# KushalChaudhari-16/Medical-Image-Denoising-Using-Diffusion

Measured on AMD Instinct MI355X. Metric: denoised images/sec, 256x256 x50 DDIM steps, higher is better.
Workload: dtype f32 (split-fp16 x3 MFMA, fp32 accumulate); 1 GPU; batch=8/GPU 256x256 grayscale, 50-iteration reverse loop (noise_steps=50, inference_steps=50), random-init 12.8M-param UNet (BASELINE.json configs[1]); batch_per_gpu=8, global_batch=8, parallelism=single, collective=none

## Files before the change

include/midd.h:

```cpp
#ifndef MIDD_H
#define MIDD_H

#include <stddef.h>
#include <stdint.h>

#ifdef __cplusplus
extern "C" {
#endif

#define MI_OK            0
#define MI_EINVAL       -1
#define MI_ESTATE       -2
#define MI_EHIP         -3
#define MI_ENOMEM       -4
#define MI_ERANGE       -5

#define MI_STATUS_NONFINITE   1
#define MI_STATUS_FP16_RANGE  2

#define MI_MAX_LEVELS    8

#define MI_VARIANT_DDIM  0
#define MI_VARIANT_CDDPM 1

// ... 198 lines not shown

int mi_denoise_tiled_self_ensemble(mi_plan* plan, const float* noisy, float* mean_out, float* std_out, float* samples_out, float* tiles_out,
                                   int B, int H, int W, int th, int tw, int oy, int ox, const int32_t* views, int n_views,
                                   const int32_t* t_list, int n_iters,
                                   const float* beta, const float* alpha, const float* alpha_hat, int noise_steps,
                                   int seeded, uint64_t seed, int64_t sample_offset, int64_t member_offset, int pass_samples, int flags,
                                   const mi_update_rule* rule, void* workspace, size_t workspace_bytes, void* stream);

size_t mi_tiled_self_ensemble_workspace_bytes(mi_plan* plan, int B, int n_views, int H, int W, int th, int tw, int oy, int ox,
                                              int pass_samples, int tiles_external);

int mi_denoise_slots_rule(mi_plan* plan, const float* cond, float* x, int B, int H, int W,
                          const int32_t* t_rows, int n_rows, const int32_t* iter_base, const int64_t* sample_index,
                          const int64_t* member, const uint32_t* frame,
                          const int32_t* t_before, const int32_t* t_after, float* x0_hist,
                          const float* beta, const float* alpha, const float* alpha_hat, int noise_steps,
                          const float* step_noise, int seeded, uint64_t seed, int flags,
                          const mi_update_rule* rule, void* workspace, size_t workspace_bytes, void* stream);

int mi_status(const void* workspace, void* stream, int* flags);

int mi_debug_fetch(mi_plan* plan, const char* module_name, int B, int H, int W,
                   const void* workspace, float* dst, int* C, int* h, int* w, void* stream);

int mi_debug_attention_split(int N, int B, int* ksplit, int* tiles_per_split);

int mi_debug_plan_dump(mi_plan* plan, int B, int H, int W, int side_by_side, char* buf, size_t cap);

int mi_debug_conv16_geometry(int ks, int stride, int tw, int mt, int nt, int wm, int wn, int cb,
                             int* ring, int* ppw, int* apw, int* lds_bytes);
int mi_debug_conv16_geometry_planes(int ks, int stride, int tw, int mt, int nt, int wm, int wn, int cb, int planes,
                                    int* ring, int* ppw, int* apw, int* lds_bytes);
int mi_debug_conv16_steps(int Cin, int ks, int cb);

const char* mi_source_hash(void);

typedef struct mi_profile_entry {
    char   name[128];
    int64_t launches;
    double total_ms;
    double flops;
    double bytes;
} mi_profile_entry;
int mi_profile_begin(mi_plan* plan);
int mi_profile_end(mi_plan* plan, mi_profile_entry* out, int max_entries, int* n_entries);

int mi_noise_images(const float* clean, const int32_t* t, const float* alpha_hat, int noise_steps,
                    const float* eps, int seeded, uint64_t seed, int64_t sample_offset, int64_t draw,
                    const int64_t* sample_index, const int64_t* draws,
                    float* x_t, float* eps_out, int B, int C, int H, int W, void* stream);
size_t mi_loss_workspace_bytes(int B, int C, int H, int W);
int mi_loss_terms(const float* clean, const float* x_t, const float* eps, const float* eps_pred,
                  const int32_t* t, const float* alpha_hat, int noise_steps,
                  int seeded, uint64_t seed, int64_t sample_offset, int64_t draw,
                  const int64_t* sample_index, const int64_t* draws, int flags, double edge_weight,
                  double* out, float* maps, int B, int C, int H, int W,
                  void* workspace, size_t workspace_bytes, void* stream);
size_t mi_denoising_loss_workspace_bytes(mi_plan* plan, int B, int H, int W);
int mi_denoising_loss(mi_plan* plan, const float* clean, const float* cond, const int32_t* t,
                      const float* alpha_hat, int noise_steps,
                      const float* eps, int seeded, uint64_t seed, int64_t sample_offset, int64_t draw,
                      const int64_t* sample_index, const int64_t* draws, int flags, double edge_weight,
                      double* out, float* maps, int B, int H, int W,
                      void* workspace, size_t workspace_bytes, void* stream);

void mi_plan_destroy(mi_plan* plan);
// ... 37 lines not shown
```

medical-image-denoising-using-diffusion_amd/csrc/in_conv.hip:

```cpp
#include "midd_internal.h"
#include "pointwise_common.h"

namespace midd {

__global__ __launch_bounds__(256)
void in_conv_kernel(const float* __restrict__ x, const float* __restrict__ cond, const float* __restrict__ w,
                    const float* __restrict__ bias, float* __restrict__ out, stat_word* __restrict__ tot, int rep, int bs,
                    int ic, int H, int W, int Cout, int rows, int blocked) {
    extern __shared__ float wl[];
    const int nw = 9 * 2 * ic * Cout;
    for (int i = threadIdx.x; i < nw + Cout; i += 256) wl[i] = (i < nw) ? w[i] : bias[i - nw];
    __syncthreads();
    const int CG = Cout >> 4;
    const int ppi = 256 / CG;
    const int tid = threadIdx.x;
    const int pl = tid / CG, cg = tid - pl * CG;
    const bool active = pl < ppi;
    const int b = blockIdx.y, row = blockIdx.x;
    const int HW = H * W;
    const int per = (HW + rows - 1) / rows;
    const int p0 = row * per, p1 = min(HW, p0 + per);
    float ssum[16], ssq[16];
#pragma unroll
    for (int k = 0; k < 16; ++k) { ssum[k] = 0.f; ssq[k] = 0.f; }
// ... 19 lines not shown
#else
                        const float v = plane[(size_t)gy * W + gx];
#endif
                        const float* wr = &wl[((dy * 3 + dx) * 2 * ic + ci) * Cout + cg * 16];
#if defined(PW_ABL) && PW_ABL == 4
                        acc[dx] += v;
#else
#pragma unroll
                        for (int k = 0; k < 4; ++k) acc[k] += v * *reinterpret_cast<const f32x4*>(wr + k * 4);
#endif
                    }
                }
            }
#pragma unroll
            for (int k = 0; k < 4; ++k) {
#if defined(PW_ABL) && PW_ABL == 1
                if (acc[k][0] == 12345.678f)
#endif
                *reinterpret_cast<f32x4*>(out + act_index(blocked, b, Cout, HW, p, cg * 16 + k * 4)) = acc[k];
#if !(defined(PW_ABL) && PW_ABL == 2)
#pragma unroll
                for (int e = 0; e < 4; ++e) { ssum[k * 4 + e] += acc[k][e]; ssq[k * 4 + e] += acc[k][e] * acc[k][e]; }
#endif
            }
        }
    }
    if (tot == nullptr) return;
    float* const scratch = wl + nw + Cout;
    stat_word* const acc_lds = reinterpret_cast<stat_word*>(scratch + 2 * (size_t)Cout * ppi + (((nw + Cout) & 1) ? 1 : 0));
    pointwise_publish<16>(ssum, ssq, active, pl, ppi, cg, Cout, scratch, acc_lds, tot, b, bs, rep, row % rep, tid);
}

template <int COUT, bool BLOCKED>
__global__ __launch_bounds__(256, 3)
void in_conv1_kernel(const float* __restrict__ x, const float* __restrict__ cond, const float* __restrict__ w,
                     const float* __restrict__ bias, float* __restrict__ out, stat_word* __restrict__ tot, int rep, int bs,
                     int H, int W, int per) {
    constexpr int NQ = COUT / 4;
    constexpr int G64 = (NQ % 16 == 0) ? 16 : (NQ % 8 == 0) ? 8 : (NQ % 4 == 0) ? 4 : (NQ % 2 == 0) ? 2 : 1;
    constexpr int SETS = BLOCKED ? COUT / 16 : NQ / G64;
    constexpr int PS = COUT + 4;
    constexpr int SLOTS = BLOCKED ? 64 : 4 * SETS * ((64 + NQ - 1) / NQ);
    extern __shared__ __attribute__((aligned(16))) float ic1_lds[];
    const int tid = threadIdx.x, lane = tid & 63;
    const int wave = __builtin_amdgcn_readfirstlane(tid >> 6);
    float* const tile = ic1_lds + wave * (64 * PS);
    float* const wlds = ic1_lds + 4 * 64 * PS + ((COUT + 2) * STAT_WORDS * 2 + 4);
    for (int i = tid; i < 19 * COUT; i += 256) wlds[i] = (i < 18 * COUT) ? w[i] : bias[i - 18 * COUT];
    __syncthreads();
    const int b = blockIdx.y, HW = H * W;
    const int p0 = blockIdx.x * per, p1 = min(HW, p0 + per);
    const float* const xp = x + (size_t)b * HW;
    const float* const cp = cond + (size_t)b * HW;
    float ssum[SETS][4], ssq[SETS][4];
#pragma unroll
    for (int j = 0; j < SETS; ++j)
#pragma unroll
        for (int e = 0; e < 4; ++e) { ssum[j][e] = 0.f; ssq[j][e] = 0.f; }
    auto load_taps = [&](int base, float (&v)[18]) {
        const int pc = min(base + lane, HW - 1);
        const int oy = pc / W, ox = pc - oy * W;
#pragma unroll
        for (int dy = 0; dy < 3; ++dy) {
            const int gy = oy + dy - 1, cy = min(max(gy, 0), H - 1);
#pragma unroll
            for (int dx = 0; dx < 3; ++dx) {
                const int gx = ox + dx - 1, cx = min(max(gx, 0), W - 1);
                const bool in = (gy == cy) && (gx == cx);
#if defined(PW_ABL) && PW_ABL == 6
                const float a0 = (float)cx, a1 = (float)cy;
#else
                const float a0 = xp[cy * W + cx], a1 = cp[cy * W + cx];
#endif
                v[dy * 3 + dx] = in ? a0 : 0.f;
                v[9 + dy * 3 + dx] = in ? a1 : 0.f;
            }
        }
    };
    float vn[18];
    int base = p0 + wave * 64;
    if (base < p1) load_taps(base, vn);
    for (; base < p1; base += 256) {
        float v[18];
#pragma unroll
        for (int i = 0; i < 18; ++i) v[i] = vn[i];
        if (base + 256 < p1) load_taps(base + 256, vn);
        int wofs = 0;
        asm volatile("" : "+v"(wofs));
        const float* const wl = wlds + wofs;
        constexpr int NQH = NQ / 2;
#pragma unroll
        for (int h = 0; h < 2; ++h) {
            f32x4 acc[NQH], wv[2][NQH];
            auto wload = [&](int i, f32x4 (&d)[NQH]) {
#pragma unroll
                for (int q = 0; q < NQH; ++q) d[q] = *reinterpret_cast<const f32x4*>(wl + ((i % 9) * 2 + i / 9) * COUT + (h * NQH + q) * 4);
            };
#pragma unroll
            for (int q = 0; q < NQH; ++q) acc[q] = *reinterpret_cast<const f32x4*>(wl + 18 * COUT + (h * NQH + q) * 4);
            wload(0, wv[0]);
#pragma unroll
            for (int i = 0; i < 18; ++i) {
                if (i + 1 < 18) wload(i + 1, wv[(i + 1) & 1]);
                {
                    typedef float f32x2 __attribute__((ext_vector_type(2)));
                    f32x2 tp = {v[i], v[i]};
#pragma unroll
                    for (int q = 0; q < NQH; ++q) {
                        f32x2 a0 = {acc[q][0], acc[q][1]}, a1 = {acc[q][2], acc[q][3]};
                        const f32x2 w0 = {wv[i & 1][q][0], wv[i & 1][q][1]}, w1 = {wv[i & 1][q][2], wv[i & 1][q][3]};
                        asm volatile("v_pk_fma_f32 %0, %1, %2, %0 op_sel_hi:[1,0,1]" : "+v"(a0) : "v"(w0), "v"(tp));
                        asm volatile("v_pk_fma_f32 %0, %1, %2, %0 op_sel_hi:[1,0,1]" : "+v"(a1) : "v"(w1), "v"(tp));
                        acc[q] = (f32x4){a0[0], a0[1], a1[0], a1[1]};
                    }
                }
#pragma unroll
                for (int q = 0; q < NQH; ++q) asm volatile("" : "+v"(acc[q]));
            }
#pragma unroll
            for (int q = 0; q < NQH; ++q) *reinterpret_cast<f32x4*>(&tile[lane * PS + (h * NQH + q) * 4]) = acc[q];
        }
        const int npx = min(64, p1 - base);
#pragma unroll
        for (int r = 0; r < NQ; ++r) {
            int px, c, set; float* dst;
            if constexpr (BLOCKED) {
                const int k = r >> 2, idx = (r & 3) * 64 + lane;
                px = idx >> 2; c = k * 4 + (idx & 3); set = k;
                dst = out + (((size_t)b * (COUT / 16) + k) * HW + base) * 16 + (size_t)idx * 4;
            } else {
                const int idx = r * 64 + lane;
                px = idx / NQ; c = idx - px * NQ; set = r % SETS;
                dst = out + ((size_t)b * HW + base) * COUT + (size_t)idx * 4;
            }
            const f32x4 val = *reinterpret_cast<const f32x4*>(&tile[px * PS + c * 4]);
            if (px < npx) {
#if defined(PW_ABL) && PW_ABL == 5
                if (val[0] == 12345.678f)
#endif
                *reinterpret_cast<f32x4*>(dst) = val;
#pragma unroll
                for (int e = 0; e < 4; ++e) { ssum[set][e] += val[e]; ssq[set][e] += val[e] * val[e]; }
            }
        }
    }
    if (tot == nullptr) return;
#if defined(PW_ABL) && PW_ABL == 8
    if (ssum[0][0] != 12345.678f) return;
#endif
    __syncthreads();
    float* const scratch = ic1_lds;
    for (int i = tid; i < 2 * COUT * SLOTS; i += 256) scratch[i] = 0.f;
    __syncthreads();
#pragma unroll
    for (int j = 0; j < SETS; ++j) {
        const int quad = BLOCKED ? j * 4 + (lane & 3) : (lane + 64 * j) % NQ;
        const int slot = BLOCKED ? wave * 16 + (lane >> 2) : (wave * SETS + j) * ((64 + NQ - 1) / NQ) + lane / NQ;
#pragma unroll
        for (int e = 0; e < 4; ++e) {
            scratch[(size_t)(quad * 4 + e) * SLOTS + slot] = ssum[j][e];
            scratch[(size_t)(COUT + quad * 4 + e) * SLOTS + slot] = ssq[j][e];
        }
    }
    auto fold = [&](int i) {
        double t = 0;
        for (int l = 0; l < SLOTS; ++l) t += (double)scratch[(size_t)i * SLOTS + l];
        return (float)t;
    };
    stat_word* const acc_lds = reinterpret_cast<stat_word*>(ic1_lds + 4 * 64 * PS);
    stat_publish(tot, b, COUT, bs, rep, blockIdx.x % rep, 0, COUT, fold, acc_lds, tid, 256);
}

template <int COUT, bool BLOCKED>
static hipError_t in_conv1_launch(const float* x, const float* cond, const float* w, const float* bias, float* out,
                                  stat_word* tot, int rep, int bs, int B, int H, int W, hipStream_t s) {
#ifndef IC1_PASSES
#define IC1_PASSES 2
#endif
    const int HW = H * W;
    int per = IC1_PASSES * 256;
    while ((HW + per - 1) / per > 1024) per += 256;
    const int rows = (HW + per - 1) / per;
    constexpr int NQ = COUT / 4, PS = COUT + 4;
    constexpr int G64 = (NQ % 16 == 0) ? 16 : (NQ % 8 == 0) ? 8 : (NQ % 4 == 0) ? 4 : (NQ % 2 == 0) ? 2 : 1;
    constexpr int SLOTS = BLOCKED ? 64 : 4 * (NQ / G64) * ((64 + NQ - 1) / NQ);
    static_assert(2 * COUT * SLOTS <= 4 * 64 * PS, "the statistics scratch aliases the tiles");
    const size_t lds = (size_t)4 * 64 * PS * sizeof(float) + (size_t)(COUT + 2) * STAT_WORDS * sizeof(stat_word) + 16 + (size_t)19 * COUT * sizeof(float);
    {
        static int raised[MIDD_MAX_DEVICES] = {};
        hipError_t e = ensure_dynamic_lds(reinterpret_cast<const void*>(&in_conv1_kernel<COUT, BLOCKED>), (int)lds, raised);
        if (e != hipSuccess) return e;
    }
    hipLaunchKernelGGL((in_conv1_kernel<COUT, BLOCKED>), dim3(rows, B), dim3(256), lds, s, x, cond, w, bias, out, tot, rep, bs, H, W, per);
    return hipGetLastError();
}

hipError_t in_conv_launch(const float* x, const float* cond, const float* w, const float* bias, float* out,
                          stat_word* tot, int rep, int bs, int B, int ic, int H, int W, int Cout, int blocked, hipStream_t s) {
    if (Cout % 16 || Cout / 16 > 256) return hipErrorInvalidValue;
    if (ic == 1 && in_conv1_width(Cout)) {
#define MIDD_IC1(N) if (Cout == N) return blocked ? in_conv1_launch<N, true>(x, cond, w, bias, out, tot, rep, bs, B, H, W, s) \
                                                 : in_conv1_launch<N, false>(x, cond, w, bias, out, tot, rep, bs, B, H, W, s);
        MIDD_IC1(48) MIDD_IC1(32) MIDD_IC1(64)
        static_assert(in_conv1_width(48) && in_conv1_width(32) && in_conv1_width(64), "in_conv1_width names the instantiations");
#undef MIDD_IC1
    }
    const int ppi = 256 / (Cout / 16);
    const int rows = pointwise_rows(H * W, ppi);
    const size_t lds = in_conv_lds_bytes(ic, Cout);
    if (lds > POINTWISE_LDS_LIMIT) return hipErrorInvalidValue;
    hipLaunchKernelGGL(in_conv_kernel, dim3(rows, B), dim3(256), lds, s, x, cond, w, bias, out, tot, rep, bs, ic, H, W, Cout, rows, blocked);
    return hipGetLastError();
}

}
```

medical-image-denoising-using-diffusion_amd/csrc/midd_abi.hip:

```cpp
#include "midd_host.h"

using namespace midd;

static thread_local char g_err[512] = "";

int midd::fail(int code, const char* fmt, ...) {
    va_list ap;
    va_start(ap, fmt);
    vsnprintf(g_err, sizeof(g_err), fmt, ap);
    va_end(ap);
    return code;
}

extern "C" size_t mi_resize_workspace_bytes(int n, int sw, int sh, int dw, int dh) {
    if (n < 1 || sw < 1 || sh < 1 || dw < 1 || dh < 1) return 0;
    return resize_workspace_bytes(n, sw, sh, dw, dh);
}
extern "C" int mi_resize_bicubic_u8(const void* src, int n, int sw, int sh, void* dst, int dw, int dh,
                                    void* workspace, size_t workspace_bytes, void* stream) {
    if (!src || !dst || !workspace) return fail(MI_EINVAL, "null argument");
    if (n < 1 || sw < 1 || sh < 1 || dw < 1 || dh < 1) return fail(MI_EINVAL, "image sizes must be positive");
    if (reinterpret_cast<uintptr_t>(workspace) & 255) return fail(MI_EINVAL, "workspace must be 256-byte aligned");
    if (workspace_bytes < resize_workspace_bytes(n, sw, sh, dw, dh))
        return fail(MI_EINVAL, "workspace too small: %zu < %zu", workspace_bytes, resize_workspace_bytes(n, sw, sh, dw, dh));
// ... 201 lines not shown
    if (host & ~(MI_STATUS_NONFINITE | MI_STATUS_FP16_RANGE))
        return fail(MI_ERANGE, "status word 0x%x (bit 4: a -DMIDD_DMA_CHECK build saw an operand that had not landed when its counted wait returned)", host);
    if (host & MI_STATUS_FP16_RANGE)
        return fail(MI_ERANGE, "an attention operand exceeds the split-fp16 range (|q|, |k| or |v| >= 4094, or not finite): use compute=\"f32\"%s",
                    (host & MI_STATUS_NONFINITE) ? "; non-finite values reached later statistics" : "");
    if (host & MI_STATUS_NONFINITE) return fail(MI_ERANGE, "non-finite activations (NaN / Inf) reached a GroupNorm statistic or a raw operand");
    return MI_OK;
}

extern "C" int mi_debug_conv16_geometry(int ks, int stride, int tw, int mt, int nt, int wm, int wn, int cb, int* ring, int* ppw, int* apw, int* lds_bytes) {
    if (!ring || !ppw || !apw || !lds_bytes) return fail(MI_EINVAL, "null argument");
    ConvTile t{ks, stride, tw, mt, nt, wm, wn, cb};
    ConvLaunchInfo li{};
    if (!conv16_launch_info(384, 16 * nt * wn, 1, 64, 64, t, 0, &li)) return fail(MI_EINVAL, "tile (%d,%d,%d,%d,%d) ks %d stride %d cb %d is not instantiated", tw, mt, nt, wm, wn, ks, stride, cb);
    *ring = li.ring; *ppw = li.ppw; *apw = li.apw; *lds_bytes = li.lds_bytes;
    return MI_OK;
}
extern "C" int mi_debug_conv16_geometry_planes(int ks, int stride, int tw, int mt, int nt, int wm, int wn, int cb, int planes,
                                               int* ring, int* ppw, int* apw, int* lds_bytes) {
    if (!ring || !ppw || !apw || !lds_bytes) return fail(MI_EINVAL, "null argument");
    if (planes != 1 && planes != 2) return fail(MI_EINVAL, "planes must be 1 (f16) or 2 (f16x3), got %d", planes);
    ConvTile t{ks, stride, tw, mt, nt, wm, wn, cb, planes};
    ConvLaunchInfo li{};
    if (!conv16_launch_info(384, 16 * nt * wn, 1, 64, 64, t, 0, &li)) return fail(MI_EINVAL, "tile (%d,%d,%d,%d,%d) ks %d stride %d cb %d is not instantiated", tw, mt, nt, wm, wn, ks, stride, cb);
    *ring = li.ring; *ppw = li.ppw; *apw = li.apw; *lds_bytes = li.lds_bytes;
    return MI_OK;
}
extern "C" int mi_debug_conv16_steps(int Cin, int ks, int cb) {
    if (Cin < 16 || Cin % 16) return fail(MI_EINVAL, "Cin %d: a positive multiple of 16", Cin);
    if (ks != 1 && ks != 3) return fail(MI_EINVAL, "ks %d: 1 or 3", ks);
    if (cb < 0 || cb > 2 || (ks == 1 && cb == 1)) return fail(MI_EINVAL, "cb %d: 0 (default), 1 (3x3) or 2", cb);
    return conv16_num_steps(Cin, ks * ks, cb);
}
extern "C" int mi_debug_plan_dump(mi_plan* plan, int B, int H, int W, int side_by_side, char* buf, size_t cap) {
    if (!plan) return fail(MI_EINVAL, "null plan");
    std::string text;
    int rc = dump_program(plan, B, H, W, side_by_side != 0, &text);
    if (rc) return rc;
    if (buf && cap) { snprintf(buf, cap, "%s", text.c_str()); }
    return (int)text.size();
}

extern "C" void mi_plan_destroy(mi_plan* plan) {
    if (!plan) return;
    for (auto& sp : plan->spans) { (void)hipEventDestroy(sp.a); (void)hipEventDestroy(sp.b); }
    for (hipEvent_t ev : plan->event_pool) (void)hipEventDestroy(ev);
    if (plan->sev_fork) (void)hipEventDestroy(plan->sev_fork);
    for (int i = 0; i < mi_plan::MAX_PARTS; ++i) {
        if (plan->sev_phase[i]) (void)hipEventDestroy(plan->sev_phase[i]);
        if (plan->sev_join[i]) (void)hipEventDestroy(plan->sev_join[i]);
        if (plan->sstream[i]) (void)hipStreamDestroy(plan->sstream[i]);
    }
    if (plan->wdev) (void)hipFree(plan->wdev);
    if (plan->ttab) (void)hipFree(plan->ttab);
    delete plan;
}
```

medical-image-denoising-using-diffusion_amd/csrc/pointwise_common.h:

```cpp
#pragma once
#include "midd_internal.h"

namespace midd {

typedef float f32x4 __attribute__((ext_vector_type(4)));

static inline bool aligned16(const void* p) { return (reinterpret_cast<uintptr_t>(p) & 15) == 0; }

template <int NV>
__device__ __forceinline__ void pointwise_publish(const float (&sum)[NV], const float (&sq)[NV], bool active, int pl, int ppi, int cgrp,
                                                  int C, float* scratch, stat_word* acc, stat_word* tot, int b, int bs, int rep,
                                                  int replica, int tid, int nthreads = 256, int c0 = 0, int ncol = -1) {
    if (ncol < 0) ncol = C;
    if (active) {
#pragma unroll
        for (int e = 0; e < NV; ++e) {
            scratch[(size_t)(cgrp * NV + e) * ppi + pl] = sum[e];
            scratch[(size_t)(ncol + cgrp * NV + e) * ppi + pl] = sq[e];
        }
    }
    auto fold = [&](int i) {
        double t = 0;
        for (int l = 0; l < ppi; ++l) t += (double)scratch[(size_t)i * ppi + l];
        return (float)t;
    };
    stat_publish(tot, b, C, bs, rep, replica, c0, ncol, fold, acc, tid, nthreads);
}

static inline int pointwise_rows(int HW, int ppi) {
    int r = (HW + ppi * 4 - 1) / (ppi * 4);
    return r < 1 ? 1 : (r > 1024 ? 1024 : r);
}

__device__ __forceinline__ double add_rn64(double a, double b) {
#pragma clang fp contract(off)
    return a + b;
}
__device__ __forceinline__ double sub_rn64(double a, double b) {
#pragma clang fp contract(off)
    return a - b;
}
__device__ __forceinline__ double mul_rn64(double a, double b) {
#pragma clang fp contract(off)
    return a * b;
}

}
```

medical-image-denoising-using-diffusion_amd/csrc/resample.hip:

```cpp
#include "midd_internal.h"
#include "pointwise_common.h"

namespace midd {

__global__ __launch_bounds__(256)
void resize_bilinear_kernel(const float* __restrict__ src, float* __restrict__ dst, stat_word* __restrict__ tot, int rep, int bs,
                            int H, int W, int C, int OH, int OW, float sy, float sx, int rows) {
    extern __shared__ float rs_lds[];
    const int CQ = C >> 2;
    const int ppi = 256 / CQ;
    const int tid = threadIdx.x;
    const int pl = tid / CQ, cq = tid - pl * CQ;
    const bool active = pl < ppi;
    const int b = blockIdx.y, row = blockIdx.x;
    const int OHW = OH * OW;
    const int per = (OHW + rows - 1) / rows;
    const int p0 = row * per, p1 = min(OHW, p0 + per);
    float ssum[4] = {0.f, 0.f, 0.f, 0.f}, ssq[4] = {0.f, 0.f, 0.f, 0.f};
    if (active) {
        const float* base = src + (size_t)b * H * W * C + cq * 4;
        for (int p = p0 + pl; p < p1; p += ppi) {
            const int oy = p / OW, ox = p - oy * OW;
            float fy = sy * ((float)oy + 0.5f) - 0.5f; if (fy < 0.f) fy = 0.f;
            float fx = sx * ((float)ox + 0.5f) - 0.5f; if (fx < 0.f) fx = 0.f;
            const int y0 = (int)fy, x0 = (int)fx;
            const int y1 = y0 + (y0 < H - 1 ? 1 : 0), x1 = x0 + (x0 < W - 1 ? 1 : 0);
            const float ly1 = fy - (float)y0, lx1 = fx - (float)x0;
            const float ly0 = 1.0f - ly1, lx0 = 1.0f - lx1;
            const f32x4 v00 = *reinterpret_cast<const f32x4*>(base + ((size_t)y0 * W + x0) * C);
            const f32x4 v01 = *reinterpret_cast<const f32x4*>(base + ((size_t)y0 * W + x1) * C);
            const f32x4 v10 = *reinterpret_cast<const f32x4*>(base + ((size_t)y1 * W + x0) * C);
            const f32x4 v11 = *reinterpret_cast<const f32x4*>(base + ((size_t)y1 * W + x1) * C);
            const f32x4 r = ly0 * (lx0 * v00 + lx1 * v01) + ly1 * (lx0 * v10 + lx1 * v11);
            *reinterpret_cast<f32x4*>(dst + ((size_t)b * OHW + p) * C + cq * 4) = r;
#pragma unroll
            for (int e = 0; e < 4; ++e) { ssum[e] += r[e]; ssq[e] += r[e] * r[e]; }
        }
    }
    if (tot == nullptr) return;
    stat_word* const acc_lds = reinterpret_cast<stat_word*>(rs_lds + 2 * (size_t)C * ppi);
    pointwise_publish<4>(ssum, ssq, active, pl, ppi, cq, C, rs_lds, acc_lds, tot, b, bs, rep, row % rep, tid);
}

__global__ __launch_bounds__(256)
void resize_bilinear_blocked_kernel(const float* __restrict__ src, float* __restrict__ dst, stat_word* __restrict__ tot, int rep, int bs,
                                    int H, int W, int C, int OH, int OW, float sy, float sx, int rows) {
    __shared__ float rs_scratch[2 * 16 * 64];
    __shared__ stat_word rs_acc[(16 + 2) * STAT_WORDS];
    const int tid = threadIdx.x;
    const int pl = tid >> 2, q = tid & 3;
    const int b = blockIdx.y, row = blockIdx.x, blk = blockIdx.z;
    const int OHW = OH * OW;
    const int per = (OHW + rows - 1) / rows;
    const int p0 = row * per, p1 = min(OHW, p0 + per);
    float ssum[4] = {0.f, 0.f, 0.f, 0.f}, ssq[4] = {0.f, 0.f, 0.f, 0.f};
    const float* base = src + (((size_t)b * (C >> 4) + blk) * (size_t)(H * W)) * 16 + q * 4;
    float* const obase = dst + (((size_t)b * (C >> 4) + blk) * (size_t)OHW) * 16 + q * 4;
    for (int p = p0 + pl; p < p1; p += 64) {
        const int oy = p / OW, ox = p - oy * OW;
        float fy = sy * ((float)oy + 0.5f) - 0.5f; if (fy < 0.f) fy = 0.f;
        float fx = sx * ((float)ox + 0.5f) - 0.5f; if (fx < 0.f) fx = 0.f;
        const int y0 = (int)fy, x0 = (int)fx;
        const int y1 = y0 + (y0 < H - 1 ? 1 : 0), x1 = x0 + (x0 < W - 1 ? 1 : 0);
        const float ly1 = fy - (float)y0, lx1 = fx - (float)x0;
        const float ly0 = 1.0f - ly1, lx0 = 1.0f - lx1;
        const f32x4 v00 = *reinterpret_cast<const f32x4*>(base + ((size_t)y0 * W + x0) * 16);
        const f32x4 v01 = *reinterpret_cast<const f32x4*>(base + ((size_t)y0 * W + x1) * 16);
        const f32x4 v10 = *reinterpret_cast<const f32x4*>(base + ((size_t)y1 * W + x0) * 16);
        const f32x4 v11 = *reinterpret_cast<const f32x4*>(base + ((size_t)y1 * W + x1) * 16);
        const f32x4 r = ly0 * (lx0 * v00 + lx1 * v01) + ly1 * (lx0 * v10 + lx1 * v11);
        *reinterpret_cast<f32x4*>(obase + (size_t)p * 16) = r;
#pragma unroll
        for (int e = 0; e < 4; ++e) { ssum[e] += r[e]; ssq[e] += r[e] * r[e]; }
    }
    if (tot == nullptr) return;
    pointwise_publish<4>(ssum, ssq, true, pl, 64, q, C, rs_scratch, rs_acc, tot, b, bs, rep, row % rep, tid, 256, blk * 16, 16);
}

hipError_t resize_bilinear_launch(const float* src, float* dst, stat_word* tot, int rep, int bs, int B, int H, int W, int C, int OH, int OW, int blocked, hipStream_t s) {
    if (blocked) {
        if (C % 16) return hipErrorInvalidValue;
        const int rows_b = pointwise_rows(OH * OW, 64);
        hipLaunchKernelGGL(resize_bilinear_blocked_kernel, dim3(rows_b, B, C / 16), dim3(256), 0, s,
                           src, dst, tot, rep, bs, H, W, C, OH, OW, (float)H / (float)OH, (float)W / (float)OW, rows_b);
        return hipGetLastError();
    }
    if (C % 4 || C / 4 > 256) return hipErrorInvalidValue;
    const int ppi = 256 / (C / 4);
    const int rows = pointwise_rows(OH * OW, ppi);
    const size_t lds = (size_t)2 * C * ppi * sizeof(float) + (size_t)(C + 2) * STAT_WORDS * sizeof(stat_word);
    if (lds > 64 * 1024) return hipErrorInvalidValue;
    hipLaunchKernelGGL(resize_bilinear_kernel, dim3(rows, B), dim3(256), lds, s,
                       src, dst, tot, rep, bs, H, W, C, OH, OW, (float)H / (float)OH, (float)W / (float)OW, rows);
    return hipGetLastError();
}

__global__ __launch_bounds__(256)
void conv_transpose_kernel(const float* __restrict__ src, const float* __restrict__ w, const float* __restrict__ bias,
                           float* __restrict__ dst, int B, int H, int W, int Cin, int Cout, int blocked) {
    const int OH = 2 * H, OW = 2 * W, CQ = Cout >> 2;
    const long total = (long)B * OH * OW * CQ;
    const long gid = (long)blockIdx.x * 256 + threadIdx.x;
    if (gid >= total) return;
    const int cq = (int)(gid % CQ);
    const long pix = gid / CQ;
    const int ox = (int)(pix % OW);
    const int oy = (int)((pix / OW) % OH);
    const int b = (int)(pix / ((long)OW * OH));
    f32x4 acc = *reinterpret_cast<const f32x4*>(bias + cq * 4);
    for (int ky = 0; ky < 4; ++ky) {
        const int ny = oy + 1 - ky;
        if (ny < 0 || (ny & 1) || (ny >> 1) >= H) continue;
        for (int kx = 0; kx < 4; ++kx) {
            const int nx = ox + 1 - kx;
            if (nx < 0 || (nx & 1) || (nx >> 1) >= W) continue;
// ... 54 lines not shown
```

medical-image-denoising-using-diffusion_amd/native.py:

```python
from __future__ import annotations

import ctypes as C
import os
import threading

_HERE = os.path.dirname(os.path.abspath(__file__))
LIB_PATH = os.environ.get("MIDD_LIBRARY") or os.path.join(_HERE, "libmidd.so")

MI_MAX_LEVELS = 8
MI_VARIANT = {"ddim": 0, "cddpm": 1}
MI_CLAMP_EPS = 1
MI_NO_SPLIT = 2
MI_COMPUTE = {"f32": 0, "f16x3": 1, "f16": 2}
MI_STATUS_NONFINITE, MI_STATUS_FP16_RANGE = 1, 2
MI_COMPUTE_BATCH_INVARIANT = 0x100
MI_UPDATE = {"reference": 0, "ddim": 1, "dpmpp2m": 2}
MI_PIX_U8, MI_PIX_U16, MI_PIX_F32 = 0, 1, 2


class NativeLibraryError(RuntimeError):
    pass


class MiddError(RuntimeError):
# ... 93 lines not shown
    ("mi_denoise_rule", C.c_int, [C.c_void_p, C.c_void_p, C.c_void_p, C.c_int, C.c_int, C.c_int,
                                  C.POINTER(C.c_int32), C.c_int, C.POINTER(C.c_float), C.POINTER(C.c_float),
                                  C.POINTER(C.c_float), C.c_int, C.c_void_p, C.c_int, C.c_uint64, C.c_int64, C.c_int,
                                  C.POINTER(UpdateRule), C.c_void_p, C.c_size_t, C.c_void_p]),
    ("mi_denoise_ensemble_rule", C.c_int, [C.c_void_p, C.c_void_p, C.c_void_p, C.c_void_p, C.c_void_p, C.c_int, C.c_int, C.c_int, C.c_int,
                                           C.POINTER(C.c_int32), C.c_int, C.POINTER(C.c_float), C.POINTER(C.c_float),
                                           C.POINTER(C.c_float), C.c_int, C.c_uint64, C.c_int64, C.c_int64, C.c_int, C.c_int,
                                           C.POINTER(UpdateRule), C.c_void_p, C.c_size_t, C.c_void_p]),
    ("mi_denoise_tiled_rule", C.c_int, [C.c_void_p, C.c_void_p, C.c_void_p, C.c_void_p] + [C.c_int] * 7 +
                                       [C.POINTER(C.c_int32), C.c_int, C.POINTER(C.c_float), C.POINTER(C.c_float), C.POINTER(C.c_float), C.c_int,
                                        C.c_int, C.c_uint64, C.c_int64, C.c_int, C.c_int, C.POINTER(UpdateRule), C.c_void_p, C.c_size_t, C.c_void_p]),
    ("mi_dpm_coefficients", C.c_int, [C.POINTER(C.c_int32), C.c_int, C.POINTER(C.c_float), C.c_int, C.POINTER(C.c_float)]),
    ("mi_denoise_dpm", C.c_int, [C.c_void_p, C.c_void_p, C.c_void_p, C.c_void_p, C.c_int, C.c_int, C.c_int, C.c_int,
                                 C.POINTER(C.c_int32), C.c_int, C.POINTER(C.c_float), C.POINTER(C.c_float),
                                 C.POINTER(C.c_float), C.c_int, C.c_int, C.c_int, C.c_void_p, C.c_size_t, C.c_void_p]),
    ("mi_denoise_tiled_dpm", C.c_int, [C.c_void_p, C.c_void_p, C.c_void_p, C.c_void_p, C.c_void_p] + [C.c_int] * 7 +
                                      [C.POINTER(C.c_int32), C.c_int, C.POINTER(C.c_float), C.POINTER(C.c_float), C.POINTER(C.c_float), C.c_int,
                                       C.c_int, C.c_int, C.c_int, C.c_void_p, C.c_size_t, C.c_void_p]),
    ("mi_update_row", C.c_int, [C.c_int32, C.c_int32, C.c_int32, C.POINTER(C.c_float), C.c_int, C.c_double, C.POINTER(C.c_float)]),
    ("mi_denoise_slots_rule", C.c_int, [C.c_void_p, C.c_void_p, C.c_void_p, C.c_int, C.c_int, C.c_int,
                                        C.POINTER(C.c_int32), C.c_int, C.POINTER(C.c_int32), C.POINTER(C.c_int64),
                                        C.POINTER(C.c_int64), C.POINTER(C.c_uint32),
                                        C.POINTER(C.c_int32), C.POINTER(C.c_int32), C.c_void_p,
                                        C.POINTER(C.c_float), C.POINTER(C.c_float), C.POINTER(C.c_float), C.c_int,
                                        C.c_void_p, C.c_int, C.c_uint64, C.c_int, C.POINTER(UpdateRule), C.c_void_p, C.c_size_t, C.c_void_p]),
    ("mi_debug_fetch", C.c_int, [C.c_void_p, C.c_char_p, C.c_int, C.c_int, C.c_int, C.c_void_p, C.c_void_p,
                                 C.POINTER(C.c_int), C.POINTER(C.c_int), C.POINTER(C.c_int), C.c_void_p]),
    ("mi_status", C.c_int, [C.c_void_p, C.c_void_p, C.POINTER(C.c_int)]),
    ("mi_debug_attention_split", C.c_int, [C.c_int, C.c_int, C.POINTER(C.c_int), C.POINTER(C.c_int)]),
    ("mi_debug_plan_dump", C.c_int, [C.c_void_p, C.c_int, C.c_int, C.c_int, C.c_int, C.c_char_p, C.c_size_t]),
    ("mi_debug_conv16_geometry", C.c_int, [C.c_int] * 8 + [C.POINTER(C.c_int)] * 4),
    ("mi_debug_conv16_geometry_planes", C.c_int, [C.c_int] * 9 + [C.POINTER(C.c_int)] * 4),
    ("mi_debug_conv16_steps", C.c_int, [C.c_int] * 3),
    ("mi_source_hash", C.c_char_p, []),
    ("mi_profile_begin", C.c_int, [C.c_void_p]),
    ("mi_profile_end", C.c_int, [C.c_void_p, C.POINTER(ProfileEntry), C.c_int, C.POINTER(C.c_int)]),
    ("mi_resize_workspace_bytes", C.c_size_t, [C.c_int, C.c_int, C.c_int, C.c_int, C.c_int]),
    ("mi_resize_bicubic_u8", C.c_int, [C.c_void_p, C.c_int, C.c_int, C.c_int, C.c_void_p, C.c_int, C.c_int,
                                       C.c_void_p, C.c_size_t, C.c_void_p]),
    ("mi_u8_to_unit_f32", C.c_int, [C.c_void_p, C.c_void_p, C.c_size_t, C.c_void_p]),
    ("mi_unit_f32_to_u8", C.c_int, [C.c_void_p, C.c_void_p, C.c_size_t, C.c_void_p]),
    ("mi_resize_f32_workspace_bytes", C.c_size_t, [C.c_int, C.c_int, C.c_int, C.c_int, C.c_int]),
    ("mi_resize_bicubic_f32", C.c_int, [C.c_void_p, C.c_int, C.c_int, C.c_int, C.c_int, C.c_void_p, C.c_int, C.c_int, C.c_int, C.c_int,
                                        C.c_void_p, C.c_size_t, C.c_void_p]),
    ("mi_u16_to_unit_f32", C.c_int, [C.c_void_p, C.c_void_p, C.c_size_t, C.c_void_p]),
    ("mi_unit_f32_to_u16", C.c_int, [C.c_void_p, C.c_void_p, C.c_size_t, C.c_void_p]),
    ("mi_histogram_u16", C.c_int, [C.c_void_p, C.c_int, C.c_size_t, C.c_void_p, C.c_void_p]),
    ("mi_window_levels", C.c_int, [C.c_void_p, C.c_int, C.c_double, C.c_double, C.c_void_p, C.c_void_p]),
    ("mi_window_u16_to_f32", C.c_int, [C.c_void_p, C.c_void_p, C.c_int, C.c_size_t, C.c_void_p, C.c_void_p]),
    ("mi_window_f32_to_u16", C.c_int, [C.c_void_p, C.c_void_p, C.c_int, C.c_size_t, C.c_void_p, C.c_void_p]),
    ("mi_resize_bicubic_f32_window", C.c_int, [C.c_void_p, C.c_int, C.c_int, C.c_int, C.c_int, C.c_void_p, C.c_int, C.c_int, C.c_int,
                                               C.c_int, C.c_void_p, C.c_void_p, C.c_size_t, C.c_void_p]),
    ("mi_metrics_workspace_bytes", C.c_size_t, [C.c_int, C.c_int]),
    ("mi_image_metrics", C.c_int, [C.c_void_p, C.c_void_p, C.c_int, C.c_int, C.c_int, C.c_void_p,
                                   C.c_void_p, C.c_size_t, C.c_void_p]),
    ("mi_noise_images", C.c_int, [C.c_void_p, C.POINTER(C.c_int32), C.POINTER(C.c_float), C.c_int, C.c_void_p, C.c_int, C.c_uint64, C.c_int64,
                                  C.c_int64, C.POINTER(C.c_int64), C.POINTER(C.c_int64), C.c_void_p, C.c_void_p] + [C.c_int] * 4 + [C.c_void_p]),
    ("mi_loss_workspace_bytes", C.c_size_t, [C.c_int] * 4),
    ("mi_loss_terms", C.c_int, [C.c_void_p] * 4 + [C.POINTER(C.c_int32), C.POINTER(C.c_float), C.c_int, C.c_int, C.c_uint64, C.c_int64, C.c_int64,
                                C.POINTER(C.c_int64), C.POINTER(C.c_int64), C.c_int, C.c_double, C.c_void_p, C.c_void_p] + [C.c_int] * 4 + [C.c_void_p, C.c_size_t, C.c_void_p]),
    ("mi_denoising_loss_workspace_bytes", C.c_size_t, [C.c_void_p, C.c_int, C.c_int, C.c_int]),
    ("mi_denoising_loss", C.c_int, [C.c_void_p] * 3 + [C.POINTER(C.c_int32), C.POINTER(C.c_float), C.c_int, C.c_void_p, C.c_int, C.c_uint64, C.c_int64,
                                    C.c_int64, C.POINTER(C.c_int64), C.POINTER(C.c_int64), C.c_int, C.c_double, C.c_void_p, C.c_void_p] + [C.c_int] * 3 + [C.c_void_p, C.c_size_t, C.c_void_p]),
    ("mi_plan_destroy", None, [C.c_void_p]),
    ("mi_last_error", C.c_char_p, []),
    ("mi_version", C.c_char_p, []),
# ... 47 lines not shown
```

Measured before the change: 51.09 images/s.

## Add banded 2x bilinear upsample path and dual-strip blocked first conv

Adds a specialized path for exact 2x bilinear upsampling in the blocked layout. Each block processes a band of output rows and reuses horizontally interpolated source rows held in registers, instead of recomputing the taps for every output pixel. The blocked first-conv kernel now processes two 64-pixel strips per wave so each LDS weight load is shared across both strips; its occupancy bound drops from 3 to 2 to make room for the extra registers. The statistics scratch stride is padded to an odd value to avoid LDS bank conflicts, and a debug entry point for the resize kernel is exposed.

```diff
diff --git a/include/midd.h b/include/midd.h
--- a/include/midd.h
+++ b/include/midd.h
@@ -254,6 +254,9 @@
 int mi_debug_conv16_geometry_planes(int ks, int stride, int tw, int mt, int nt, int wm, int wn, int cb, int planes,
                                     int* ring, int* ppw, int* apw, int* lds_bytes);
 int mi_debug_conv16_steps(int Cin, int ks, int cb);
+
+int mi_debug_resize_bilinear(const float* src, float* dst, uint64_t* totals, int rep, int bs, int B, int H, int W, int C,
+                             int OH, int OW, void* stream);
 
 const char* mi_source_hash(void);
 
diff --git a/medical-image-denoising-using-diffusion_amd/csrc/in_conv.hip b/medical-image-denoising-using-diffusion_amd/csrc/in_conv.hip
--- a/medical-image-denoising-using-diffusion_amd/csrc/in_conv.hip
+++ b/medical-image-denoising-using-diffusion_amd/csrc/in_conv.hip
@@ -75,7 +75,7 @@
 }
 
 template <int COUT, bool BLOCKED>
-__global__ __launch_bounds__(256, 3)
+__global__ __launch_bounds__(256, BLOCKED ? 2 : 3)
 void in_conv1_kernel(const float* __restrict__ x, const float* __restrict__ cond, const float* __restrict__ w,
                      const float* __restrict__ bias, float* __restrict__ out, stat_word* __restrict__ tot, int rep, int bs,
                      int H, int W, int per) {
@@ -120,70 +120,139 @@
             }
         }
     };
-    float vn[18];
-    int base = p0 + wave * 64;
-    if (base < p1) load_taps(base, vn);
-    for (; base < p1; base += 256) {
-        float v[18];
-#pragma unroll
-        for (int i = 0; i < 18; ++i) v[i] = vn[i];
-        if (base + 256 < p1) load_taps(base + 256, vn);
-        int wofs = 0;
-        asm volatile("" : "+v"(wofs));
-        const float* const wl = wlds + wofs;
-        constexpr int NQH = NQ / 2;
-#pragma unroll
-        for (int h = 0; h < 2; ++h) {
-            f32x4 acc[NQH], wv[2][NQH];
-            auto wload = [&](int i, f32x4 (&d)[NQH]) {
-#pragma unroll
-                for (int q = 0; q < NQH; ++q) d[q] = *reinterpret_cast<const f32x4*>(wl + ((i % 9) * 2 + i / 9) * COUT + (h * NQH + q) * 4);
-            };
-#pragma unroll
-            for (int q = 0; q < NQH; ++q) acc[q] = *reinterpret_cast<const f32x4*>(wl + 18 * COUT + (h * NQH + q) * 4);
-            wload(0, wv[0]);
-#pragma unroll
-            for (int i = 0; i < 18; ++i) {
-                if (i + 1 < 18) wload(i + 1, wv[(i + 1) & 1]);
-                {
-                    typedef float f32x2 __attribute__((ext_vector_type(2)));
-                    f32x2 tp = {v[i], v[i]};
-#pragma unroll
-                    for (int q = 0; q < NQH; ++q) {
-                        f32x2 a0 = {acc[q][0], acc[q][1]}, a1 = {acc[q][2], acc[q][3]};
-                        const f32x2 w0 = {wv[i & 1][q][0], wv[i & 1][q][1]}, w1 = {wv[i & 1][q][2], wv[i & 1][q][3]};
-                        asm volatile("v_pk_fma_f32 %0, %1, %2, %0 op_sel_hi:[1,0,1]" : "+v"(a0) : "v"(w0), "v"(tp));
-                        asm volatile("v_pk_fma_f32 %0, %1, %2, %0 op_sel_hi:[1,0,1]" : "+v"(a1) : "v"(w1), "v"(tp));
-                        acc[q] = (f32x4){a0[0], a0[1], a1[0], a1[1]};
+    if constexpr (BLOCKED) {
+        constexpr int NB = COUT / 16;
+        float vn[2][18];
+        int base = p0 + wave * 64;
+        if (base < p1) { load_taps(base, vn[0]); load_taps(base + 256, vn[1]); }
+        for (; base < p1; base += 512) {
+            float v[2][18];
+#pragma unroll
+            for (int s = 0; s < 2; ++s)
+#pragma unroll
+                for (int i = 0; i < 18; ++i) v[s][i] = vn[s][i];
+            if (base + 512 < p1) { load_taps(base + 512, vn[0]); load_taps(base + 768, vn[1]); }
+            int wofs = 0;
+            asm volatile("" : "+v"(wofs));
+            const float* const wl = wlds + wofs;
+#pragma unroll
+            for (int k = 0; k < NB; ++k) {
+                f32x4 acc[2][4], wv[2][4];
+                auto wload = [&](int i, f32x4 (&d)[4]) {
+#pragma unroll
+                    for (int q = 0; q < 4; ++q) d[q] = *reinterpret_cast<const f32x4*>(wl + ((i % 9) * 2 + i / 9) * COUT + (k * 4 + q) * 4);
+                };
+#pragma unroll
+                for (int q = 0; q < 4; ++q) acc[0][q] = acc[1][q] = *reinterpret_cast<const f32x4*>(wl + 18 * COUT + (k * 4 + q) * 4);
+                wload(0, wv[0]);
+#pragma unroll
+                for (int i = 0; i < 18; ++i) {
+                    if (i + 1 < 18) wload(i + 1, wv[(i + 1) & 1]);
+#pragma unroll
+                    for (int s = 0; s < 2; ++s) {
+                        typedef float f32x2 __attribute__((ext_vector_type(2)));
+                        f32x2 tp = {v[s][i], v[s][i]};
+#pragma unroll
+                        for (int q = 0; q < 4; ++q) {
+                            f32x2 a0 = {acc[s][q][0], acc[s][q][1]}, a1 = {acc[s][q][2], acc[s][q][3]};
+                            const f32x2 w0 = {wv[i & 1][q][0], wv[i & 1][q][1]}, w1 = {wv[i & 1][q][2], wv[i & 1][q][3]};
+                            asm volatile("v_pk_fma_f32 %0, %1, %2, %0 op_sel_hi:[1,0,1]" : "+v"(a0) : "v"(w0), "v"(tp));
+                            asm volatile("v_pk_fma_f32 %0, %1, %2, %0 op_sel_hi:[1,0,1]" : "+v"(a1) : "v"(w1), "v"(tp));
+                            acc[s][q] = (f32x4){a0[0], a0[1], a1[0], a1[1]};
+                        }
                     }
-                }
-#pragma unroll
-                for (int q = 0; q < NQH; ++q) asm volatile("" : "+v"(acc[q]));
-            }
-#pragma unroll
-            for (int q = 0; q < NQH; ++q) *reinterpret_cast<f32x4*>(&tile[lane * PS + (h * NQH + q) * 4]) = acc[q];
-        }
-        const int npx = min(64, p1 - base);
-#pragma unroll
-        for (int r = 0; r < NQ; ++r) {
-            int px, c, set; float* dst;
-            if constexpr (BLOCKED) {
-                const int k = r >> 2, idx = (r & 3) * 64 + lane;
-                px = idx >> 2; c = k * 4 + (idx & 3); set = k;
-                dst = out + (((size_t)b * (COUT / 16) + k) * HW + base) * 16 + (size_t)idx * 4;
-            } else {
-                const int idx = r * 64 + lane;
-                px = idx / NQ; c = idx - px * NQ; set = r % SETS;
-                dst = out + ((size_t)b * HW + base) * COUT + (size_t)idx * 4;
-            }
-            const f32x4 val = *reinterpret_cast<const f32x4*>(&tile[px * PS + c * 4]);
-            if (px < npx) {
+#pragma unroll
+                    for (int s = 0; s < 2; ++s)
+#pragma unroll
+                        for (int q = 0; q < 4; ++q) asm volatile("" : "+v"(acc[s][q]));
+                }
+#pragma unroll
+                for (int s = 0; s < 2; ++s) {
+                    const int sbase = base + 256 * s, npx = min(64, p1 - sbase);
+#pragma unroll
+                    for (int q = 0; q < 4; ++q) *reinterpret_cast<f32x4*>(&tile[lane * PS + (k * 4 + q) * 4]) = acc[s][q];
+#pragma unroll
+                    for (int r4 = 0; r4 < 4; ++r4) {
+                        const int idx = r4 * 64 + lane, px = idx >> 2, c = k * 4 + (idx & 3);
+                        const f32x4 val = *reinterpret_cast<const f32x4*>(&tile[px * PS + c * 4]);
+                        if (px < npx) {
 #if defined(PW_ABL) && PW_ABL == 5
-                if (val[0] == 12345.678f)
-#endif
-                *reinterpret_cast<f32x4*>(dst) = val;
-#pragma unroll
-                for (int e = 0; e < 4; ++e) { ssum[set][e] += val[e]; ssq[set][e] += val[e] * val[e]; }
+                            if (val[0] == 12345.678f)
+#endif
+                            *reinterpret_cast<f32x4*>(out + (((size_t)b * NB + k) * HW + sbase) * 16 + (size_t)idx * 4) = val;
+#pragma unroll
+                            for (int e = 0; e < 4; ++e) { ssum[k][e] += val[e]; ssq[k][e] += val[e] * val[e]; }
+                        }
+                    }
+                }
+            }
+        }
+    } else {
+        float vn[18];
+        int base = p0 + wave * 64;
+        if (base < p1) load_taps(base, vn);
+        for (; base < p1; base += 256) {
+            float v[18];
+#pragma unroll
+            for (int i = 0; i < 18; ++i) v[i] = vn[i];
+            if (base + 256 < p1) load_taps(base + 256, vn);
+            int wofs = 0;
+            asm volatile("" : "+v"(wofs));
+            const float* const wl = wlds + wofs;
+            constexpr int NQH = NQ / 2;
+#pragma unroll
+            for (int h = 0; h < 2; ++h) {
+                f32x4 acc[NQH], wv[2][NQH];
+                auto wload = [&](int i, f32x4 (&d)[NQH]) {
+#pragma unroll
+                    for (int q = 0; q < NQH; ++q) d[q] = *reinterpret_cast<const f32x4*>(wl + ((i % 9) * 2 + i / 9) * COUT + (h * NQH + q) * 4);
+                };
+#pragma unroll
+                for (int q = 0; q < NQH; ++q) acc[q] = *reinterpret_cast<const f32x4*>(wl + 18 * COUT + (h * NQH + q) * 4);
+                wload(0, wv[0]);
+#pragma unroll
+                for (int i = 0; i < 18; ++i) {
+                    if (i + 1 < 18) wload(i + 1, wv[(i + 1) & 1]);
+                    {
+                        typedef float f32x2 __attribute__((ext_vector_type(2)));
+                        f32x2 tp = {v[i], v[i]};
+#pragma unroll
+                        for (int q = 0; q < NQH; ++q) {
+                            f32x2 a0 = {acc[q][0], acc[q][1]}, a1 = {acc[q][2], acc[q][3]};
+                            const f32x2 w0 = {wv[i & 1][q][0], wv[i & 1][q][1]}, w1 = {wv[i & 1][q][2], wv[i & 1][q][3]};
+                            asm volatile("v_pk_fma_f32 %0, %1, %2, %0 op_sel_hi:[1,0,1]" : "+v"(a0) : "v"(w0), "v"(tp));
+                            asm volatile("v_pk_fma_f32 %0, %1, %2, %0 op_sel_hi:[1,0,1]" : "+v"(a1) : "v"(w1), "v"(tp));
+                            acc[q] = (f32x4){a0[0], a0[1], a1[0], a1[1]};
+                        }
+                    }
+#pragma unroll
+                    for (int q = 0; q < NQH; ++q) asm volatile("" : "+v"(acc[q]));
+                }
+#pragma unroll
+                for (int q = 0; q < NQH; ++q) *reinterpret_cast<f32x4*>(&tile[lane * PS + (h * NQH + q) * 4]) = acc[q];
+            }
+            const int npx = min(64, p1 - base);
+#pragma unroll
+            for (int r = 0; r < NQ; ++r) {
+                int px, c, set; float* dst;
+                if constexpr (BLOCKED) {
+                    const int k = r >> 2, idx = (r & 3) * 64 + lane;
+                    px = idx >> 2; c = k * 4 + (idx & 3); set = k;
+                    dst = out + (((size_t)b * (COUT / 16) + k) * HW + base) * 16 + (size_t)idx * 4;
+                } else {
+                    const int idx = r * 64 + lane;
+                    px = idx / NQ; c = idx - px * NQ; set = r % SETS;
+                    dst = out + ((size_t)b * HW + base) * COUT + (size_t)idx * 4;
+                }
+                const f32x4 val = *reinterpret_cast<const f32x4*>(&tile[px * PS + c * 4]);
+                if (px < npx) {
+#if defined(PW_ABL) && PW_ABL == 5
+                    if (val[0] == 12345.678f)
+#endif
+                    *reinterpret_cast<f32x4*>(dst) = val;
+#pragma unroll
+                    for (int e = 0; e < 4; ++e) { ssum[set][e] += val[e]; ssq[set][e] += val[e] * val[e]; }
+                }
             }
         }
     }
@@ -193,7 +262,8 @@
 #endif
     __syncthreads();
     float* const scratch = ic1_lds;
-    for (int i = tid; i < 2 * COUT * SLOTS; i += 256) scratch[i] = 0.f;
+    constexpr int SSTR = SLOTS | 1;
+    for (int i = tid; i < 2 * COUT * SSTR; i += 256) scratch[i] = 0.f;
     __syncthreads();
 #pragma unroll
     for (int j = 0; j < SETS; ++j) {
@@ -201,13 +271,13 @@
         const int slot = BLOCKED ? wave * 16 + (lane >> 2) : (wave * SETS + j) * ((64 + NQ - 1) / NQ) + lane / NQ;
 #pragma unroll
         for (int e = 0; e < 4; ++e) {
-            scratch[(size_t)(quad * 4 + e) * SLOTS + slot] = ssum[j][e];
-            scratch[(size_t)(COUT + quad * 4 + e) * SLOTS + slot] = ssq[j][e];
+            scratch[(size_t)(quad * 4 + e) * SSTR + slot] = ssum[j][e];
+            scratch[(size_t)(COUT + quad * 4 + e) * SSTR + slot] = ssq[j][e];
         }
     }
     auto fold = [&](int i) {
         double t = 0;
-        for (int l = 0; l < SLOTS; ++l) t += (double)scratch[(size_t)i * SLOTS + l];
+        for (int l = 0; l < SLOTS; ++l) t += (double)scratch[(size_t)i * SSTR + l];
         return (float)t;
     };
     stat_word* const acc_lds = reinterpret_cast<stat_word*>(ic1_lds + 4 * 64 * PS);
@@ -227,7 +297,7 @@
     constexpr int NQ = COUT / 4, PS = COUT + 4;
     constexpr int G64 = (NQ % 16 == 0) ? 16 : (NQ % 8 == 0) ? 8 : (NQ % 4 == 0) ? 4 : (NQ % 2 == 0) ? 2 : 1;
     constexpr int SLOTS = BLOCKED ? 64 : 4 * (NQ / G64) * ((64 + NQ - 1) / NQ);
-    static_assert(2 * COUT * SLOTS <= 4 * 64 * PS, "the statistics scratch aliases the tiles");
+    static_assert(2 * COUT * (SLOTS | 1) <= 4 * 64 * PS, "the statistics scratch aliases the tiles");
     const size_t lds = (size_t)4 * 64 * PS * sizeof(float) + (size_t)(COUT + 2) * STAT_WORDS * sizeof(stat_word) + 16 + (size_t)19 * COUT * sizeof(float);
     {
         static int raised[MIDD_MAX_DEVICES] = {};
diff --git a/medical-image-denoising-using-diffusion_amd/csrc/midd_abi.hip b/medical-image-denoising-using-diffusion_amd/csrc/midd_abi.hip
--- a/medical-image-denoising-using-diffusion_amd/csrc/midd_abi.hip
+++ b/medical-image-denoising-using-diffusion_amd/csrc/midd_abi.hip
@@ -257,6 +257,14 @@
     if (cb < 0 || cb > 2 || (ks == 1 && cb == 1)) return fail(MI_EINVAL, "cb %d: 0 (default), 1 (3x3) or 2", cb);
     return conv16_num_steps(Cin, ks * ks, cb);
 }
+extern "C" int mi_debug_resize_bilinear(const float* src, float* dst, uint64_t* totals, int rep, int bs, int B, int H, int W, int C, int OH, int OW, void* stream) {
+    if (!src || !dst) return fail(MI_EINVAL, "null tensor");
+    if (B < 1 || H < 1 || W < 1 || OH < 1 || OW < 1 || C < 16 || C % 16) return fail(MI_EINVAL, "B %d, %dx%d -> %dx%d, C %d: positive sizes, C a multiple of 16", B, H, W, OH, OW, C);
+    if (totals && (rep < 1 || rep > STAT_MAX_REPLICAS || bs < 1 || C % bs)) return fail(MI_EINVAL, "rep %d (1..%d), bs %d (a divisor of C = %d)", rep, STAT_MAX_REPLICAS, bs, C);
+    if ((long long)B * C * H * W >= (1ll << 31) || (long long)B * C * OH * OW >= (1ll << 31)) return fail(MI_EINVAL, "tensor of 2^31 elements or more");
+    HIPCHK(resize_bilinear_launch(src, dst, reinterpret_cast<stat_word*>(totals), totals ? rep : 1, totals ? bs : C, B, H, W, C, OH, OW, 1, static_cast<hipStream_t>(stream)));
+    return MI_OK;
+}
 extern "C" int mi_debug_plan_dump(mi_plan* plan, int B, int H, int W, int side_by_side, char* buf, size_t cap) {
     if (!plan) return fail(MI_EINVAL, "null plan");
     std::string text;
diff --git a/medical-image-denoising-using-diffusion_amd/csrc/pointwise_common.h b/medical-image-denoising-using-diffusion_amd/csrc/pointwise_common.h
--- a/medical-image-denoising-using-diffusion_amd/csrc/pointwise_common.h
+++ b/medical-image-denoising-using-diffusion_amd/csrc/pointwise_common.h
@@ -10,18 +10,19 @@
 template <int NV>
 __device__ __forceinline__ void pointwise_publish(const float (&sum)[NV], const float (&sq)[NV], bool active, int pl, int ppi, int cgrp,
                                                   int C, float* scratch, stat_word* acc, stat_word* tot, int b, int bs, int rep,
-                                                  int replica, int tid, int nthreads = 256, int c0 = 0, int ncol = -1) {
+                                                  int replica, int tid, int nthreads = 256, int c0 = 0, int ncol = -1, int sstr = -1) {
+    if (sstr < 0) sstr = ppi;
     if (ncol < 0) ncol = C;
     if (active) {
 #pragma unroll
         for (int e = 0; e < NV; ++e) {
-            scratch[(size_t)(cgrp * NV + e) * ppi + pl] = sum[e];
-            scratch[(size_t)(ncol + cgrp * NV + e) * ppi + pl] = sq[e];
+            scratch[(size_t)(cgrp * NV + e) * sstr + pl] = sum[e];
+            scratch[(size_t)(ncol + cgrp * NV + e) * sstr + pl] = sq[e];
         }
     }
     auto fold = [&](int i) {
         double t = 0;
-        for (int l = 0; l < ppi; ++l) t += (double)scratch[(size_t)i * ppi + l];
+        for (int l = 0; l < ppi; ++l) t += (double)scratch[(size_t)i * sstr + l];
         return (float)t;
     };
     stat_publish(tot, b, C, bs, rep, replica, c0, ncol, fold, acc, tid, nthreads);
diff --git a/medical-image-denoising-using-diffusion_amd/csrc/resample.hip b/medical-image-denoising-using-diffusion_amd/csrc/resample.hip
--- a/medical-image-denoising-using-diffusion_amd/csrc/resample.hip
+++ b/medical-image-denoising-using-diffusion_amd/csrc/resample.hip
@@ -42,20 +42,76 @@
     pointwise_publish<4>(ssum, ssq, active, pl, ppi, cq, C, rs_lds, acc_lds, tot, b, bs, rep, row % rep, tid);
 }
 
+#ifndef MIDD_RS2X_ROWS
+#define MIDD_RS2X_ROWS 16
+#endif
+constexpr int RS2X_ROWS = MIDD_RS2X_ROWS;
+__host__ __device__ static inline bool resize_is_2x(int H, int W, int OH, int OW) { return OH == 2 * H && OW == 2 * W; }
+
+__device__ __forceinline__ void resize2x_band(const float* __restrict__ base, float* __restrict__ obase, int H, int W, int OH, int OW,
+                                              float sy, float sx, int pl, float (&ssum)[4], float (&ssq)[4]) {
+#pragma clang fp contract(off)
+    constexpr int NR = RS2X_ROWS / 2 + 2;
+    const int strips = (OW + 63) >> 6;
+    const int band = blockIdx.x / strips, strip = blockIdx.x - band * strips;
+    const int ox = strip * 64 + pl;
+    const bool live = ox < OW;
+    float fx = sx * ((float)min(ox, OW - 1) + 0.5f) - 0.5f; if (fx < 0.f) fx = 0.f;
+    const int x0 = (int)fx, x1 = x0 + (x0 < W - 1 ? 1 : 0);
+    const float lx1 = fx - (float)x0, lx0 = 1.0f - lx1;
+    const int k0 = band * (RS2X_ROWS / 2);
+    f32x4 va[NR], vb[NR];
+#pragma unroll
+    for (int t = 0; t < NR; ++t) {
+        const int y = min(max(k0 - 1 + t, 0), H - 1);
+        va[t] = *reinterpret_cast<const f32x4*>(base + ((size_t)y * W + x0) * 16);
+        vb[t] = *reinterpret_cast<const f32x4*>(base + ((size_t)y * W + x1) * 16);
+    }
+    f32x4 hl[NR];
+#pragma unroll
+    for (int t = 0; t < NR; ++t) {
+        const f32x4 m = lx0 * va[t];
+#pragma unroll
+        for (int e = 0; e < 4; ++e) hl[t][e] = __builtin_fmaf(lx1, vb[t][e], m[e]);
+    }
+#pragma unroll
+    for (int i = 0; i < RS2X_ROWS; ++i) {
+        const int oy = band * RS2X_ROWS + i;
+        if (oy >= OH) break;
+        float fy = sy * ((float)oy + 0.5f) - 0.5f; if (fy < 0.f) fy = 0.f;
+        const float ly1 = fy - (float)(int)fy, ly0 = 1.0f - ly1;
+        const int t0 = (i >> 1) + (i & 1);
+        const f32x4 top = (i == 0 && oy == 0) ? hl[1] : hl[t0];
+        const f32x4 bot = (i == 0 && oy == 0) ? hl[2] : hl[t0 + 1];
+        const f32x4 m = ly1 * bot;
+        f32x4 r;
+#pragma unroll
+        for (int e = 0; e < 4; ++e) r[e] = __builtin_fmaf(ly0, top[e], m[e]);
+        if (live) *reinterpret_cast<f32x4*>(obase + ((size_t)oy * OW + ox) * 16) = r;
+#pragma unroll
+        for (int e = 0; e < 4; ++e) {
+            const float v = live ? r[e] : 0.f;
+            ssum[e] += v; ssq[e] = __builtin_fmaf(v, v, ssq[e]);
+        }
+    }
+}
+
 __global__ __launch_bounds__(256)
 void resize_bilinear_blocked_kernel(const float* __restrict__ src, float* __restrict__ dst, stat_word* __restrict__ tot, int rep, int bs,
                                     int H, int W, int C, int OH, int OW, float sy, float sx, int rows) {
-    __shared__ float rs_scratch[2 * 16 * 64];
+    __shared__ float rs_scratch[2 * 16 * 65];
     __shared__ stat_word rs_acc[(16 + 2) * STAT_WORDS];
     const int tid = threadIdx.x;
     const int pl = tid >> 2, q = tid & 3;
     const int b = blockIdx.y, row = blockIdx.x, blk = blockIdx.z;
     const int OHW = OH * OW;
     const int per = (OHW + rows - 1) / rows;
-    const int p0 = row * per, p1 = min(OHW, p0 + per);
+    const bool x2 = resize_is_2x(H, W, OH, OW);
+    const int p0 = row * per, p1 = x2 ? p0 : min(OHW, p0 + per);
     float ssum[4] = {0.f, 0.f, 0.f, 0.f}, ssq[4] = {0.f, 0.f, 0.f, 0.f};
     const float* base = src + (((size_t)b * (C >> 4) + blk) * (size_t)(H * W)) * 16 + q * 4;
     float* const obase = dst + (((size_t)b * (C >> 4) + blk) * (size_t)OHW) * 16 + q * 4;
+    if (x2) resize2x_band(base, obase, H, W, OH, OW, sy, sx, pl, ssum, ssq);
     for (int p = p0 + pl; p < p1; p += 64) {
         const int oy = p / OW, ox = p - oy * OW;
         float fy = sy * ((float)oy + 0.5f) - 0.5f; if (fy < 0.f) fy = 0.f;
@@ -74,13 +130,16 @@
         for (int e = 0; e < 4; ++e) { ssum[e] += r[e]; ssq[e] += r[e] * r[e]; }
     }
     if (tot == nullptr) return;
-    pointwise_publish<4>(ssum, ssq, true, pl, 64, q, C, rs_scratch, rs_acc, tot, b, bs, rep, row % rep, tid, 256, blk * 16, 16);
+#if defined(PW_ABL) && PW_ABL == 21
+    if (ssum[0] != 12345.678f) return;
+#endif
+    pointwise_publish<4>(ssum, ssq, true, pl, 64, q, C, rs_scratch, rs_acc, tot, b, bs, rep, row % rep, tid, 256, blk * 16, 16, 65);
 }
 
 hipError_t resize_bilinear_launch(const float* src, float* dst, stat_word* tot, int rep, int bs, int B, int H, int W, int C, int OH, int OW, int blocked, hipStream_t s) {
     if (blocked) {
         if (C % 16) return hipErrorInvalidValue;
-        const int rows_b = pointwise_rows(OH * OW, 64);
+        const int rows_b = resize_is_2x(H, W, OH, OW) ? ((OW + 63) / 64) * ((OH + RS2X_ROWS - 1) / RS2X_ROWS) : pointwise_rows(OH * OW, 64);
         hipLaunchKernelGGL(resize_bilinear_blocked_kernel, dim3(rows_b, B, C / 16), dim3(256), 0, s,
                            src, dst, tot, rep, bs, H, W, C, OH, OW, (float)H / (float)OH, (float)W / (float)OW, rows_b);
         return hipGetLastError();
diff --git a/medical-image-denoising-using-diffusion_amd/native.py b/medical-image-denoising-using-diffusion_amd/native.py
--- a/medical-image-denoising-using-diffusion_amd/native.py
+++ b/medical-image-denoising-using-diffusion_amd/native.py
@@ -149,6 +149,7 @@
     ("mi_debug_conv16_geometry", C.c_int, [C.c_int] * 8 + [C.POINTER(C.c_int)] * 4),
     ("mi_debug_conv16_geometry_planes", C.c_int, [C.c_int] * 9 + [C.POINTER(C.c_int)] * 4),
     ("mi_debug_conv16_steps", C.c_int, [C.c_int] * 3),
+    ("mi_debug_resize_bilinear", C.c_int, [C.c_void_p, C.c_void_p, C.c_void_p] + [C.c_int] * 8 + [C.c_void_p]),
     ("mi_source_hash", C.c_char_p, []),
     ("mi_profile_begin", C.c_int, [C.c_void_p]),
     ("mi_profile_end", C.c_int, [C.c_void_p, C.POINTER(ProfileEntry), C.c_int, C.POINTER(C.c_int)]),
```

Measured after the change: 51.22 images/s (median of 6 runs). Within noise of the previous version (+0.3%).
